# ysnrkdm/subproc

Measured on AMD Instinct MI355X. Metric: env-steps/sec (batched self-play), higher is better.
Workload: dtype u64

## Files before the change

subproc_amd/csrc/bitboard.hpp:

```cpp
#pragma once
#include <hip/hip_runtime.h>
#include <stdint.h>

namespace oth {

typedef uint64_t u64;
typedef uint32_t u32;

constexpr u64 INNER_FILES = 0x7E7E7E7E7E7E7E7Eull;

template <int TT>
__device__ __forceinline__ u64 bitop3(u64 a, u64 b, u64 c) {
    const u32 hi = (u32)__builtin_amdgcn_bitop3_b32((u32)(a >> 32), (u32)(b >> 32), (u32)(c >> 32), TT);
    const u32 lo = (u32)__builtin_amdgcn_bitop3_b32((u32)a, (u32)b, (u32)c, TT);
    return ((u64)hi << 32) | lo;
}
__device__ __forceinline__ u64 bfi(u64 m, u64 a, u64 b) { return bitop3<0xCA>(m, a, b); }
__device__ __forceinline__ u64 andn(u64 a, u64 b) { return bitop3<0x30>(a, b, b); }
__device__ __forceinline__ u64 or3(u64 a, u64 b, u64 c) { return bitop3<0xFE>(a, b, c); }
__device__ __forceinline__ u64 and2(u64 a, u64 b) { return bitop3<0xC0>(a, b, b); }
__device__ __forceinline__ u64 or2(u64 a, u64 b) { return bitop3<0xFC>(a, b, b); }
template <int K, bool L>
__device__ __forceinline__ u32 sh32(u32 x) {
    u32 r;
    if (L) asm("v_lshlrev_b32_e64 %0, %2, %1" : "=v"(r) : "v"(x), "i"(K));
    else asm("v_lshrrev_b32_e64 %0, %2, %1" : "=v"(r) : "v"(x), "i"(K));
    return r;
}
template <int S, bool L>
__device__ __forceinline__ u64 sh(u64 x) {
    static_assert(S > 0 && S < 64, "shift amount");
    u64 r;
    if (L) asm("v_lshlrev_b64 %0, %2, %1" : "=v"(r) : "v"(x), "i"(S));
    else asm("v_lshrrev_b64 %0, %2, %1" : "=v"(r) : "v"(x), "i"(S));
    return r;
}

struct PairProp {
    u64 pro, p2L, p4L, p2R, p4R;
};
template <int S>
__device__ __forceinline__ PairProp pair_prop(u64 pro) {
    PairProp q;
    q.pro = pro;
    q.p2L = and2(pro, sh<S, true>(pro));
    q.p4L = and2(q.p2L, sh<2 * S, true>(q.p2L));
    q.p2R = sh<S, false>(q.p2L);
    q.p4R = sh<3 * S, false>(q.p4L);
    return q;
}

template <int K, bool L>
__device__ __forceinline__ u64 ks_step(u64 gen, u64 pro) {
    if constexpr (K >= 32) {
        u32 lo = (u32)gen, hi = (u32)(gen >> 32);
        if (L) {
            const u32 s = K == 32 ? lo : sh32<(K == 32 ? 1 : K - 32), true>(lo);
            hi = (u32)__builtin_amdgcn_bitop3_b32((u32)(pro >> 32), s, hi, 0xCA);
        } else {
            const u32 s = K == 32 ? hi : sh32<(K == 32 ? 1 : K - 32), false>(hi);
            lo = (u32)__builtin_amdgcn_bitop3_b32((u32)pro, s, lo, 0xCA);
        }
        return ((u64)hi << 32) | lo;
    } else {
        return bfi(pro, sh<K, L>(gen), gen);
    }
}

template <int S, bool L>
__device__ __forceinline__ u64 ks(u64 gen, const PairProp& q) {
    gen = ks_step<S, L>(gen, q.pro);
    gen = ks_step<2 * S, L>(gen, L ? q.p2L : q.p2R);
    gen = ks_step<4 * S, L>(gen, L ? q.p4L : q.p4R);
    return gen;
}

__device__ __forceinline__ u64 lshl1_add(u64 x, u64 y) {
    u64 r;
    asm("v_lshl_add_u64 %0, %1, 1, %2" : "=v"(r) : "v"(x), "v"(y));
    return r;
}
__device__ __forceinline__ u64 add64(u64 x, u64 y) {
    u64 r;
    asm("v_lshl_add_u64 %0, %1, 0, %2" : "=v"(r) : "v"(x), "v"(y));
    return r;
}
__device__ __forceinline__ u64 dec64(u64 x) {
    u64 r;
    asm("v_lshl_add_u64 %0, %1, 0, -1" : "=v"(r) : "v"(x));
    return r;
}
__device__ __forceinline__ u64 east_run(u64 src, u64 Oi) { return andn(Oi, lshl1_add(src, Oi)); }

__device__ __forceinline__ u32 bfrev32(u32 x) {
    u32 r;
    asm("v_bfrev_b32_e64 %0, %1" : "=v"(r) : "v"(x));
    return r;
}
__device__ __forceinline__ u64 rev64(u64 x) { return ((u64)bfrev32((u32)x) << 32) | bfrev32((u32)(x >> 32)); }

struct Position {
    u64 Oi, rOi;
    u64 A[8];
    u64 reach;
    u64 legal;
};

constexpr int kFillOrder = 798;
template <int ORDER = kFillOrder>
__device__ __forceinline__ void analyse(u64 P, u64 O, Position& s) {
    const u64 Oi = and2(O, INNER_FILES);
    s.Oi = Oi;
    s.rOi = rev64(Oi);
    const PairProp v = pair_prop<8>(O), d9 = pair_prop<9>(Oi), d7 = pair_prop<7>(Oi);
    s.A[0] = east_run(P, Oi);
    s.A[1] = rev64(east_run(rev64(P), s.rOi));
    {
        constexpr int order[3] = {ORDER / 100, ORDER / 10 % 10, ORDER % 10};
#pragma unroll
        for (int k = 0; k < 3; k++) {
            if (order[k] == 8) {
                s.A[2] = and2(ks<8, true>(P, v), O);
                s.A[3] = and2(ks<8, false>(P, v), O);
            } else if (order[k] == 9) {
                s.A[4] = and2(ks<9, true>(P, d9), O);
                s.A[5] = and2(ks<9, false>(P, d9), O);
            } else {
                s.A[6] = and2(ks<7, true>(P, d7), O);
                s.A[7] = and2(ks<7, false>(P, d7), O);
            }
        }
    }
    u64 m = or3(sh<1, true>(s.A[0]), sh<1, false>(s.A[1]), sh<8, true>(s.A[2]));
    m = or3(m, sh<8, false>(s.A[3]), sh<9, true>(s.A[4]));
    m = or3(m, sh<9, false>(s.A[5]), sh<7, true>(s.A[6]));
    m = or2(m, sh<7, false>(s.A[7]));
    s.reach = m;
    s.legal = bitop3<0x04>(P, m, O);
}

constexpr int kRayRows = 6;
constexpr int kTabRows = kRayRows + 2;
__host__ __device__ inline u64 ray_from(int sq, int dx, int dy) {
    u64 r = 0;
    int x = sq & 7, y = sq >> 3;
    for (;;) {
        x += dx;
        y += dy;
        if (x < 0 || x > 7 || y < 0 || y > 7) break;
        r |= 1ull << (x + 8 * y);
    }
    return r;
}
__device__ __forceinline__ void ray_table_init(u64* tab) {
    for (int e = threadIdx.x; e < kTabRows * 64; e += blockDim.x) {
        const int row = e >> 6, sq = e & 63;
        const int dx[6] = {0, 1, -1, 0, -1, 1}, dy[6] = {1, 1, 1, -1, -1, -1};
        if (row >= kRayRows) {
            tab[e] = 1ull << (row == kRayRows ? sq : 63 - sq);
            continue;
        }
        const u64 r = ray_from(sq, dx[row], dy[row]);
        tab[e] = row < 3 ? r : rev64(r);
    }
}
__device__ __forceinline__ u64 square_bit(u32 sq, const u64* tab) { return tab[kRayRows * 64 + sq]; }
__device__ __forceinline__ u64 and3(u64 a, u64 b, u64 c) { return bitop3<0x80>(a, b, c); }
__device__ __forceinline__ u64 run_prefix(u64 R, u64 A) {
    const u64 x = andn(R, A);
    return and3(R, A, dec64(x));
}

struct RunSets {
    u64 A1, A3, A5, A7, rA0, rA2, rA4, rA6;
};
__device__ __forceinline__ RunSets run_sets(const Position& s) {
    return RunSets{s.A[1], s.A[3], s.A[5], s.A[7], rev64(s.A[0]), rev64(s.A[2]), rev64(s.A[4]), rev64(s.A[6])};
}

struct Flips {
    u64 f, fr;
};
__device__ __forceinline__ Flips flips_col(u64 mv, const RunSets& r, const u64* col) {
    const u64 rmv = col[(kRayRows + 1) * 64];
    u64 f = bitop3<0xBA>(r.A1, lshl1_add(mv, r.A1), mv);
    u64 fr = bitop3<0xBA>(r.rA0, lshl1_add(rmv, r.rA0), rmv);
    f = or3(f, run_prefix(col[0 * 64], r.A3), run_prefix(col[1 * 64], r.A5));
    f = or2(f, run_prefix(col[2 * 64], r.A7));
    fr = or3(fr, run_prefix(col[3 * 64], r.rA2), run_prefix(col[4 * 64], r.rA4));
    fr = or2(fr, run_prefix(col[5 * 64], r.rA6));
    return Flips{f, rev64(fr)};
}
__device__ __forceinline__ Flips flips_rays(u32 sq, const RunSets& r, const u64* tab) {
    return flips_col(tab[kRayRows * 64 + sq], r, tab + sq);
}
__device__ __forceinline__ void place(u64& X, u64& Y, const Flips& fl) {
    X = or3(X, fl.f, fl.fr);
    Y = bitop3<0x10>(Y, fl.f, fl.fr);
}
__device__ __forceinline__ const u64* ray_col(const u64* tab, u32 off) {
    return reinterpret_cast<const u64*>(reinterpret_cast<const char*>(tab) + off);
}

__device__ __forceinline__ u64 sel_nz(u64 t, u64 x) {
    u32 lo, hi;
    u64 m;
    asm("v_cmp_ne_u64_e64 %2, 0, %3\n\t"
        "s_nop 1\n\t"
        "v_cndmask_b32_e64 %0, 0, %4, %2\n\t"
        "v_cndmask_b32_e64 %1, 0, %5, %2"
        : "=&v"(lo), "=&v"(hi), "=&s"(m)
        : "v"(t), "v"((u32)x), "v"((u32)(x >> 32)));
    return ((u64)hi << 32) | lo;
}
__device__ __forceinline__ u64 ray_flips(u64 mv, u64 R, u64 P, u64 O) {
    const u64 sum = add64(bfi(R, O, ~0ull), mv);
    const u64 run = bitop3<0x20>(R, sum, O);
    return sel_nz(and3(sum, R, P), run);
}

__device__ __forceinline__ void rays_of(u32 sq, u64 (&R)[kRayRows]) {
    const u32 rsq = sq ^ 63u;
    R[0] = 0x0101010101010100ull << sq;
    R[1] = 0x8040201008040200ull << sq;
    R[2] = 0x0002040810204080ull << sq;
    R[3] = 0x0101010101010100ull << rsq;
    R[4] = 0x8040201008040200ull << rsq;
    R[5] = 0x0002040810204080ull << rsq;
}

__device__ __forceinline__ u64 flips_carry(u32 sq, u64 P, u64 O) {
    u64 R[kRayRows];
    rays_of(sq, R);
    const u64 mv = 1ull << sq, rmv = 1ull << (63u - sq);
    const u64 rP = rev64(P), rO = rev64(O);
    const u64 Oi = and2(O, INNER_FILES), rOi = and2(rO, INNER_FILES);
    const u64 se = lshl1_add(mv, Oi), sw = lshl1_add(rmv, rOi);
    u64 f = sel_nz(and2(se, P), andn(Oi, se));
    u64 fr = sel_nz(and2(sw, rP), andn(rOi, sw));
    f = or3(f, ray_flips(mv, R[0], P, O), ray_flips(mv, R[1], P, Oi));
    f = or2(f, ray_flips(mv, R[2], P, Oi));
    fr = or3(fr, ray_flips(rmv, R[3], rP, rO), ray_flips(rmv, R[4], rP, rOi));
    fr = or2(fr, ray_flips(rmv, R[5], rP, rOi));
    return or2(f, rev64(fr));
}

template <int ORDER = kFillOrder>
__device__ __forceinline__ u64 moves(u64 P, u64 O) {
    Position s;
    analyse<ORDER>(P, O, s);
    return s.legal;
}

__device__ __forceinline__ u64 moves_empty_side(u64 black, u64 white) {
    const u64 E = ~(black | white);
    Position s;
    analyse(E, black, s);
    return s.reach & E;
}

__device__ __forceinline__ void kth_table_init(uint8_t* tab) {
    for (int b = threadIdx.x; b < 256; b += blockDim.x) {
        int k = 0;
        for (int i = 0; i < 8; i++)
            if (b >> i & 1) tab[b * 8 + k++] = (uint8_t)i;
        for (; k < 8; k++) tab[b * 8 + k] = 0;
    }
}
__device__ __forceinline__ u32 add_lshl3(u32 a, u32 b) {
    u32 r;
    asm("v_add_lshl_u32 %0, %1, %2, 3" : "=v"(r) : "v"(a), "v"(b));
    return r;
}
template <int S, bool W>
__device__ __forceinline__ void kth_level(u32& k, u32 c, u32& off, u32& w, u32 w_hi) {
    u32 d, k2, o, w2;
    u64 b;
    if (W)
        asm("v_sub_co_u32_e64 %0, %4, %5, %6\n\t"
            "s_nop 1\n\t"
            "v_cndmask_b32_e64 %1, %0, %5, %4\n\t"
            "v_cndmask_b32_e64 %2, %7, 0, %4\n\t"
            "v_cndmask_b32_e64 %3, %9, %8, %4"
            : "=&v"(d), "=&v"(k2), "=&v"(o), "=v"(w2), "=&s"(b)
            : "v"(k), "v"(c), "i"(S), "v"(w), "v"(w_hi));
    else
        asm("v_sub_co_u32_e64 %0, %3, %4, %5\n\t"
            "s_nop 1\n\t"
            "v_cndmask_b32_e64 %1, %0, %4, %3\n\t"
            "v_cndmask_b32_e64 %2, %6, 0, %3"
            : "=&v"(d), "=&v"(k2), "=v"(o), "=&s"(b)
            : "v"(k), "v"(c), "i"(S));
    k = k2;
    off = o;
    if (W) w = w2;
}
__device__ __forceinline__ u32 kth_bit_off(u64 x, u32 k, u32 c_lo, const uint8_t* tab) {
    u32 w = (u32)x, b32, s16, s8;
    kth_level<32, true>(k, c_lo, b32, w, (u32)(x >> 32));
    kth_level<16, false>(k, __popc(w & 0xFFFFu), s16, w, 0u);
    w >>= s16;
    kth_level<8, false>(k, __popc(w & 0xFFu), s8, w, 0u);
    const u32 byte = __builtin_amdgcn_ubfe(w, s8, 8);
    const u32 lvl = (u32)__builtin_amdgcn_bitop3_b32(b32, s16, s8, 0xFE);
    return add_lshl3(lvl, tab[byte * 8u + k]);
}
__device__ __forceinline__ u32 kth_bit_tab(u64 x, u32 k, u32 c_lo, const uint8_t* tab) {
    return kth_bit_off(x, k, c_lo, tab) >> 3;
}

__device__ __forceinline__ u32 kth_bit(u64 x, u32 k) {
    u32 lo = (u32)x, hi = (u32)(x >> 32);
    u32 c = __popc(lo);
    bool up = k >= c;
    u32 w = up ? hi : lo;
    k = up ? k - c : k;
    u32 pos = up ? 32u : 0u;
#pragma unroll
    for (int half = 16; half >= 1; half >>= 1) {
        const u32 mask = (1u << half) - 1u;
        c = __popc(w & mask);
        up = k >= c;
        w = up ? (w >> half) : w;
        k = up ? k - c : k;
        pos += up ? (u32)half : 0u;
    }
    return pos;
}

}
```

subproc_amd/csrc/othello.hip:

```cpp
#include <hip/hip_runtime.h>
#include <stdint.h>
#include <stdlib.h>

#include <algorithm>
#include <climits>
#include <cmath>
#include <atomic>
#include <mutex>

#include "../../include/othello.h"
#include "bitboard.hpp"
#include "td_skey.hpp"

#define OTH_VERSION "subproc_amd 0.1.0 gfx950"

namespace {

using namespace oth;

constexpr u64 OPEN_BLACK = 0x0000000810000000ull;
constexpr u64 OPEN_WHITE = 0x0000001008000000ull;
constexpr int kBlock = 256;

constexpr u64 GOLDEN64 = 0x9E3779B97F4A7C15ull;
__host__ __device__ __forceinline__ u64 mix64(u64 z) {
    z = (z ^ (z >> 30)) * 0xBF58476D1CE4E5B9ull;
    z = (z ^ (z >> 27)) * 0x94D049BB133111EBull;
    return z ^ (z >> 31);
}
__device__ __forceinline__ u64 game_key(u64 S, u64 g) { return mix64(S + g * GOLDEN64); }
constexpr u32 LCG_MUL = 0x915F77F5u;
struct GameRng {
    u32 state, inc;
    __device__ __forceinline__ void init(u64 key) {
        state = (u32)key;
        inc = (u32)(key >> 32) | 1u;
    }
    __device__ __forceinline__ u32 pick(u32 n) {
        state = state * LCG_MUL + inc;
        return __umulhi(state, n);
    }
};
__device__ __forceinline__ u32 pick_legal(u64 legal, GameRng& rng, const uint8_t* kth_tab) {
    const u32 c_lo = __popc((u32)legal);
    return kth_bit_tab(legal, rng.pick(c_lo + __popc((u32)(legal >> 32))), c_lo, kth_tab);
}


__constant__ u64 kRegionMasks[8] = {0x8100000000000081ull, 0x4281000000008142ull, 0x0042000000004200ull,
                                    0x2400810000810024ull, 0x1800008181000018ull, 0x003C424242423C00ull,
                                    0x0000240000240000ull, 0x0000183C3C180000ull};

constexpr int kEvalRow = 12;
constexpr int kEvalTable = OTH_EVAL_PHASES * kEvalRow;
struct EvalWeights {
    int8_t w[OTH_EVAL_WEIGHTS];
};
__device__ __forceinline__ u32 eval_shard(u32 discs) { return discs ? (min(discs, 64u) - 1u) >> 4 : 0u; }
__device__ __forceinline__ void eval_weights_to_lds(const EvalWeights& ew, int* w_s) {
    for (int e = threadIdx.x; e < OTH_EVAL_PHASES * kEvalRow; e += blockDim.x) {
        const int r = e / kEvalRow, c = e % kEvalRow;
        w_s[e] = c < OTH_EVAL_FEATURES ? (int)ew.w[r * OTH_EVAL_FEATURES + c] : 0;
    }
}
__device__ __forceinline__ int eval_mul(int w, int c) { return __mul24(w, c); }
__device__ __forceinline__ int eval_linear(const int* w, u64 mine, u64 mob) {
    int v = eval_mul(w[0], (int)__popcll(mob));
#pragma unroll
    for (int k = 0; k < 8; k++) v += eval_mul(w[1 + k], (int)__popcll(and2(mine, kRegionMasks[k])));
    return v;
}

template <int POLICY>
__device__ __forceinline__ const int* child_row(u64 P, u64 O, const int* w_tab) {
    if (POLICY != OTH_POLICY_EVAL) return w_tab;
    return w_tab + kEvalRow * eval_shard((u32)__popcll(P | O) + 1u);
}
template <int POLICY>
__device__ __forceinline__ u32 child_key(u64 P, u64 O, const RunSets& s, u32 sq, const u64* rays, const int* row) {
    place(P, O, flips_rays(sq, s, rays));
    if (POLICY == OTH_POLICY_GREEDY) return ((u32)__popcll(moves(O, P)) << 6) | sq;
    int w[OTH_EVAL_FEATURES];
#pragma unroll
    for (int j = 0; j < OTH_EVAL_FEATURES; j++) w[j] = row[j];
    const int v = eval_linear(w, P, moves<798>(P, O));
    return ((u32)((1 << 20) - v) << 6) | sq;
}

template <int POLICY>
__device__ __forceinline__ u32 lane_choose(const Position& pos, u64 P, u64 O, const u64* rays, const int* w_tab) {
    u32 best = 0xFFFFFFFFu;
    u64 legal = pos.legal;
    const RunSets s = run_sets(pos);
    const int* row = child_row<POLICY>(P, O, w_tab);
    while (legal) {
        const u32 sq = (u32)__builtin_ctzll(legal);
        legal &= legal - 1;
        best = min(best, child_key<POLICY>(P, O, s, sq, rays, row));
    }
    return best & 63u;
}

struct CoopWave {
    u64 rec[64][10];
    u64 legal[64];
    u32 best[64];
};
__device__ __forceinline__ void wave_sync() {
    __builtin_amdgcn_fence(__ATOMIC_SEQ_CST, "wavefront");
    __builtin_amdgcn_wave_barrier();
}
static_assert(sizeof(RunSets) == 8 * sizeof(u64), "parent record: P, O, RunSets");
__device__ __forceinline__ void load_parent(const u64* r, u64& P, u64& O, RunSets& s) {
    P = r[0];
    O = r[1];
    s = *reinterpret_cast<const RunSets*>(r + 2);
}
__device__ __forceinline__ u32 wave_incl_scan(u32 x) {
    x += (u32)__builtin_amdgcn_update_dpp(0, (int)x, 0x111, 0xf, 0xf, false);
    x += (u32)__builtin_amdgcn_update_dpp(0, (int)x, 0x112, 0xf, 0xf, false);
    x += (u32)__builtin_amdgcn_update_dpp(0, (int)x, 0x114, 0xf, 0xf, false);
    x += (u32)__builtin_amdgcn_update_dpp(0, (int)x, 0x118, 0xf, 0xf, false);
    x += (u32)__builtin_amdgcn_update_dpp(0, (int)x, 0x142, 0xa, 0xf, false);
    x += (u32)__builtin_amdgcn_update_dpp(0, (int)x, 0x143, 0xc, 0xf, false);
    return x;
}
template <int POLICY>
__device__ u32 coop_choose(bool need, u64 P, u64 O, u32 tbl, const Position& pos, CoopWave& cw, const u64* rays,
                           const int* w_s, const uint8_t* kth_tab, u32 lane, u32 cap) {
    auto publish = [&] {
        u64* r = cw.rec[lane];
        r[0] = P;
        r[1] = O;
        RunSets rs = run_sets(pos);
        if (POLICY == OTH_POLICY_EVAL) rs.A1 |= (u64)(tbl & 1u);
        *reinterpret_cast<RunSets*>(r + 2) = rs;
    };
    constexpr bool kFirst = POLICY == OTH_POLICY_GREEDY;
    if (kFirst && need) publish();
    if (cap == 0) return need ? lane_choose<POLICY>(pos, P, O, rays, w_s + (tbl ? kEvalTable : 0)) : 64u;
    const u64 legal = need ? pos.legal : 0ull;
    const u32 cnt = (u32)__popcll(legal);
    const u32 incl = wave_incl_scan(cnt);
    const u32 T = (u32)__builtin_amdgcn_readlane((int)incl, 63);
    const u32 R = (T + 63u) >> 6;
    cw.legal[lane] = legal;
    if (need) {
        if (!kFirst) publish();
        cw.best[lane] = 0xFFFFFFFFu;
    }
    const u32 t0 = R * lane, cnt_mine = t0 < T ? min(R, T - t0) : 0u;
    const u32 excl = incl - cnt;
    const u64 with_moves = __ballot(cnt != 0);
    u32 p = 0;
#pragma unroll
    for (u32 step = 32; step >= 1; step >>= 1)
        if ((u32)__shfl((int)excl, (int)(p + step)) <= t0) p += step;
    const u32 k0 = t0 - (u32)__shfl((int)excl, (int)p);
    wave_sync();
    u64 m = 0, Pp = 0, Op = 0;
    RunSets ps = {};
    const int* row = w_s;
    auto enter = [&](u32 q) {
        load_parent(cw.rec[q], Pp, Op, ps);
        row = child_row<POLICY>(Pp, Op, w_s + ((ps.A1 & 1ull) ? kEvalTable : 0));
    };
    if (cnt_mine) {
        m = cw.legal[p];
        enter(p);
        if (k0) m &= ~0ull << kth_bit_tab(m, k0, (u32)__popc((u32)m), kth_tab);
    }
    for (u32 r = 0; r < cnt_mine; r++) {
        if (m == 0) {
            p = (u32)__ffsll((unsigned long long)(with_moves & (~0ull << (p + 1)))) - 1u;
            m = cw.legal[p];
            enter(p);
        }
        const u32 sq = (u32)__builtin_ctzll(m);
        m &= m - 1;
        atomicMin(&cw.best[p], child_key<POLICY>(Pp, Op, ps, sq, rays, row));
    }
    wave_sync();
    return need ? cw.best[lane] & 63u : 64u;
}

__device__ __forceinline__ int lane_id() { return __lane_id(); }
__device__ __forceinline__ u64 moves_of(u64 P, u64 O) { return moves(P, O); }

__global__ __launch_bounds__(kBlock) void reset_kernel(u64* __restrict__ boards, uint8_t* __restrict__ turn,
                                                       uint8_t* __restrict__ nturn, int64_t n) {
    const int64_t i = (int64_t)blockIdx.x * kBlock + threadIdx.x;
    if (i >= n) return;
    reinterpret_cast<ulonglong2*>(boards)[i] = make_ulonglong2(OPEN_BLACK, OPEN_WHITE);
    if (turn) turn[i] = OTH_BLACK;
    if (nturn) nturn[i] = 0;
}

__device__ __forceinline__ u64 legal_any(u64 bl, u64 wh, u32 t) {
    if (t == OTH_BLACK) return moves(bl, wh);
    if (t == OTH_WHITE) return moves(wh, bl);
    if (t == 0) return moves_empty_side(bl, wh);
    return 0ull;
}

struct StepOut {
    u64 bl, wh, flips;
    u32 t;
    int ret;
};
__device__ __forceinline__ StepOut put_s_any(u64 bl, u64 wh, u32 t, u32 c) {
    const u64 occ = bl | wh;
    const bool black = t == OTH_BLACK, white = t == OTH_WHITE;
    const u64 own = black ? bl : (white ? wh : (t == 0 ? ~occ : 0ull));
    const u64 opp = black ? wh : bl;
    StepOut o{bl, wh, 0ull, t, -1};
    if (c == OTH_PASS) {
        o.ret = 0;
    } else if (c < 64 && !(occ >> c & 1ull)) {
        const u64 f = flips_carry(c, own, opp);
        if (f) {
            const u64 mv = 1ull << c;
            o.ret = __popcll(f);
            o.flips = f;
            if (black) {
                o.bl = or3(bl, f, mv);
                o.wh = andn(wh, f);
            } else if (white) {
                o.wh = or3(wh, f, mv);
                o.bl = andn(bl, f);
            } else {
                o.bl = andn(bl, f);
            }
        }
    }
    if (o.ret >= 0) o.t = black ? OTH_WHITE : OTH_BLACK;
    return o;
}

__global__ __launch_bounds__(kBlock) void legal_kernel(const u64* __restrict__ boards,
                                                       const uint8_t* __restrict__ turn, u64* __restrict__ legal,
                                                       int64_t n) {
    const int64_t i = (int64_t)blockIdx.x * kBlock + threadIdx.x;
    if (i >= n) return;
    const ulonglong2 b = reinterpret_cast<const ulonglong2*>(boards)[i];
    legal[i] = legal_any(b.x, b.y, turn[i]);
}

__device__ __forceinline__ void step_board(int64_t i, ulonglong2 b, u32 t, u32 mvc, u64* boards_out, uint8_t* turn_out,
                                           u64* __restrict__ flips_out,
                                           u64* __restrict__ legal_next, int8_t* __restrict__ ret_out,
                                           uint8_t* __restrict__ nturn) {
    u64 nb, nw, f = 0, lg = 0;
    u32 t_out;
    int r = -1;
    if (t == OTH_BLACK || t == OTH_WHITE) {
        const bool black = t == OTH_BLACK;
        u64 P = black ? b.x : b.y;
        u64 O = black ? b.y : b.x;
        if (mvc == OTH_PASS) {
            r = 0;
        } else if (mvc < 64) {
            const u64 mv = 1ull << mvc;
            if (!((P | O) & mv)) {
                f = flips_carry(mvc, P, O);
                if (f) {
                    r = __popcll(f);
                    P = or3(P, f, mv);
                    O = andn(O, f);
                }
            }
        }
        const bool moved = r >= 0;
        t_out = moved ? (t ^ 3u) : t;
        if (legal_next) {
            const u64 nP = moved ? O : P, nO = moved ? P : O;
            lg = moves(nP, nO);
        }
        nb = black ? P : O;
        nw = black ? O : P;
    } else {
        const StepOut o = put_s_any(b.x, b.y, t, mvc);
        nb = o.bl;
        nw = o.wh;
        f = o.flips;
        r = o.ret;
        t_out = o.t;
        if (legal_next) lg = legal_any(nb, nw, t_out);
    }
    if (legal_next) __builtin_nontemporal_store(lg, legal_next + i);
    if (boards_out) {
        __builtin_nontemporal_store(nb, boards_out + 2 * i);
        __builtin_nontemporal_store(nw, boards_out + 2 * i + 1);
    }
    if (turn_out) __builtin_nontemporal_store((uint8_t)t_out, turn_out + i);
    if (flips_out) __builtin_nontemporal_store(f, flips_out + i);
    if (ret_out) __builtin_nontemporal_store((int8_t)r, ret_out + i);
    if (nturn && r >= 0) nturn[i] = (uint8_t)(nturn[i] + 1);
}

constexpr int kStepPerThread = 1;
__global__ __launch_bounds__(kBlock) void step_kernel(const u64* boards_in, const uint8_t* turn_in,
                                                      const uint8_t* __restrict__ move, u64* boards_out,
                                                      uint8_t* turn_out, u64* __restrict__ flips_out,
                                                      u64* __restrict__ legal_next, int8_t* __restrict__ ret_out,
                                                      uint8_t* __restrict__ nturn, int64_t n) {
    const int64_t i0 = (int64_t)blockIdx.x * kBlock + threadIdx.x, stride = (int64_t)gridDim.x * kBlock;
    ulonglong2 b[kStepPerThread];
    u32 t[kStepPerThread], mvc[kStepPerThread];
#pragma unroll
    for (int j = 0; j < kStepPerThread; j++) {
        const int64_t i = i0 + j * stride;
        if (i < n) {
            b[j] = reinterpret_cast<const ulonglong2*>(boards_in)[i];
            t[j] = turn_in[i];
            mvc[j] = move[i];
            asm volatile("" ::"v"(t[j]), "v"(mvc[j]));
        }
    }
#pragma unroll
    for (int j = 0; j < kStepPerThread; j++) {
        const int64_t i = i0 + j * stride;
        if (i < n) step_board(i, b[j], t[j], mvc[j], boards_out, turn_out, flips_out, legal_next, ret_out, nturn);
    }
}

__device__ __forceinline__ bool step_on_board(int64_t x, int64_t d, int k, int64_t& out) {
    int64_t t;
    return !__builtin_mul_overflow(d, (int64_t)k, &t) && !__builtin_add_overflow(x, t, &out) && out >= 0 && out < 8;
}
__global__ __launch_bounds__(kBlock) void hands_kernel(const u64* __restrict__ own, const u64* __restrict__ hostile,
                                                       const int64_t* __restrict__ xs, const int64_t* __restrict__ ys,
                                                       const int64_t* __restrict__ dxs,
                                                       const int64_t* __restrict__ dys,
                                                       uint8_t* __restrict__ count, int64_t n) {
    const int64_t i = (int64_t)blockIdx.x * kBlock + threadIdx.x;
    if (i >= n) return;
    const u64 mine = own[i], opp = hostile[i];
    const int64_t x = xs[i], y = ys[i], dx = dxs[i], dy = dys[i];
    int run = 0;
    for (int k = 1; k < 9; k++) {
        int64_t nx, ny;
        const bool on = step_on_board(x, dx, k, nx) && step_on_board(y, dy, k, ny);
        const u64 bit = on ? 1ull << (nx + 8 * ny) : 0ull;
        if (opp & bit) {
            run = k;
        } else {
            if (!(mine & bit)) run = 0;
            break;
        }
    }
    count[i] = (uint8_t)run;
}

__global__ __launch_bounds__(kBlock) void result_kernel(const u64* __restrict__ boards, uint8_t* __restrict__ nb,
                                                        uint8_t* __restrict__ nw, int8_t* __restrict__ diff,
                                                        uint8_t* __restrict__ terminal, int64_t n) {
    const int64_t i = (int64_t)blockIdx.x * kBlock + threadIdx.x;
    if (i >= n) return;
    const ulonglong2 b = reinterpret_cast<const ulonglong2*>(boards)[i];
    const int cb = __popcll(b.x), cw = __popcll(b.y);
    if (nb) nb[i] = (uint8_t)cb;
    if (nw) nw[i] = (uint8_t)cw;
    if (diff) diff[i] = (int8_t)(cb - cw);
    if (terminal) terminal[i] = (moves(b.x, b.y) == 0 && moves(b.y, b.x) == 0) ? 1 : 0;
}


struct RolloutArgs {
    const u64* start;
    const uint8_t* start_turn;
    u64 seed_state;
    u64 game_id0;
    int n_random;
    u64* final_boards;
    int8_t* diff;
    uint8_t* plies;
    uint8_t* moves;
    long long* hist;
    int64_t n;
    unsigned long long* work;
    u64 last_ticket;
    u32 coop_cap;
    EvalWeights ew[2];
    u32 n_rand_a, n_rand_b;
    int swap;
    uint8_t* a_black;
    u32 handoff_k;
};

constexpr u32 kHandoffK = 16;
constexpr u32 kHandoffKMax = 16;
constexpr int kPoolCap = 64 + (int)kHandoffKMax;
struct Parked {
    u64 P, O;
    u32 state, inc;
    u32 g;
    u32 bits;
};
static_assert(sizeof(Parked) == 32, "two 16-B LDS accesses per parked game");
constexpr u64 kParkedGame = ~0ull;

constexpr int kRecStride = OTH_MOVES_STRIDE + 4;
constexpr int kRecWaveBytes = 64 * kRecStride;
constexpr size_t rec_stage_bytes(int policy, bool record) {
    return record && policy == OTH_POLICY_RANDOM ? (size_t)(kBlock / 64) * kRecWaveBytes : 0;
}

constexpr int kRandomFillOrder = 789;
constexpr int rollout_waves_per_simd(int policy) { return policy == OTH_POLICY_GREEDY ? 5 : 4; }
template <int POLICY, bool RECORD, bool RUNNER = false>
__global__ __launch_bounds__(kBlock, rollout_waves_per_simd(POLICY)) void rollout_kernel(RolloutArgs a) {
    __shared__ unsigned long long hist_s[OTH_HIST_BINS];
    __shared__ uint8_t kth_tab[256 * 8];
    __shared__ u64 rays[kTabRows * 64];
    __shared__ int w_s[POLICY == OTH_POLICY_EVAL ? 2 * kEvalTable : 1];
    __shared__ CoopWave coop[POLICY == OTH_POLICY_RANDOM ? 1 : kBlock / 64];
    constexpr bool kPool = POLICY == OTH_POLICY_RANDOM && !RECORD && !RUNNER;
    __shared__ Parked pool_s[kPool ? kBlock / 64 : 1][kPool ? kPoolCap : 1];
    for (int k = threadIdx.x; k < OTH_HIST_BINS; k += kBlock) hist_s[k] = 0;
    kth_table_init(kth_tab);
    ray_table_init(rays);
    if (POLICY == OTH_POLICY_EVAL) {
        eval_weights_to_lds(a.ew[0], w_s);
        eval_weights_to_lds(a.ew[1], w_s + kEvalTable);
    }
    __syncthreads();

    const int lane = lane_id();
    const u64 n = (u64)a.n;
    u64 plies_sum = 0;
    constexpr bool kRecStage = RECORD && POLICY == OTH_POLICY_RANDOM;
    extern __shared__ u32 rec_dyn[];
    uint8_t* const rec_wave = reinterpret_cast<uint8_t*>(rec_dyn) + (threadIdx.x >> 6) * kRecWaveBytes;
    uint8_t* const rec_row = rec_wave + lane * kRecStride;

    Parked* const pool = pool_s[kPool ? threadIdx.x >> 6 : 0];
    u32 parked = 0;
    bool exhausted = false;
    (void)pool;
    (void)exhausted;
    for (;;) {
        bool from_pool = false;
        u64 base = 0;
        if (kPool && parked >= 64u) {
            from_pool = true;
        } else if (!kPool || !exhausted) {
            if (lane == 0) {
                base = atomicAdd(a.work, 64ull);
                if (base == a.last_ticket) atomicExch(a.work, 0ull);
            }
            base = __shfl(base, 0);
            if (base >= n) {
                if (!kPool || parked == 0u) break;
                exhausted = true;
                from_pool = true;
            }
        } else {
            if (parked == 0u) break;
            from_pool = true;
        }

        u64 g = base + lane;
        bool active = !from_pool && g < n;
        u64 P = OPEN_BLACK, O = OPEN_WHITE;
        u32 side = OTH_BLACK, ply = 0;
        bool passed = false;
        GameRng rng;
        if (active) {
            rng.init(game_key(a.seed_state, a.game_id0 + g));
            if (a.start) {
                const ulonglong2 s0 = reinterpret_cast<const ulonglong2*>(a.start)[g];
                side = a.start_turn ? a.start_turn[g] : OTH_BLACK;
                side = side == OTH_WHITE ? OTH_WHITE : OTH_BLACK;
                P = side == OTH_BLACK ? s0.x : s0.y;
                O = side == OTH_BLACK ? s0.y : s0.x;
            }
            if (RECORD && !kRecStage) {
                uint4* mrec = reinterpret_cast<uint4*>(a.moves + g * OTH_MOVES_STRIDE);
#pragma unroll
                for (int q = 0; q < OTH_MOVES_STRIDE / 16; q++) mrec[q] = make_uint4(~0u, ~0u, ~0u, ~0u);
            }
        }
        if constexpr (kRecStage) {
#pragma unroll
            for (int q = 0; q < OTH_MOVES_STRIDE / 4; q++) reinterpret_cast<u32*>(rec_row)[q] = ~0u;
        }
        auto rec_put = [&](u32 i, uint8_t code) {
            if (i >= OTH_MOVES_STRIDE) return;
            if constexpr (kRecStage) rec_row[i] = code;
            else a.moves[g * OTH_MOVES_STRIDE + i] = code;
        };

        if constexpr (POLICY == OTH_POLICY_RANDOM) {
            bool b0 = side == OTH_BLACK;
            u32 discs0 = RECORD ? 0u : (u32)__popcll(P | O);
            u32 npass = 0;
            if (kPool && from_pool) {
                const u32 take = min(parked, 64u);
                active = (u32)lane < take;
                if (active) {
                    const Parked e = pool[parked - take + lane];
                    P = e.P;
                    O = e.O;
                    rng.state = e.state;
                    rng.inc = e.inc;
                    g = e.g;
                    b0 = e.bits & 1u;
                    passed = (e.bits >> 1) & 1u;
                    discs0 = (e.bits >> 2) & 0x7fu;
                    npass = e.bits >> 9;
                }
                parked -= take;
            }
            const u32 hand_k = __builtin_amdgcn_readfirstlane(kPool && !from_pool ? a.handoff_k : 0u);
            const u32 parked0 = __builtin_amdgcn_readfirstlane(parked);
            (void)hand_k;
            (void)parked0;
            auto ply_of = [&](u64& X, u64& Y) -> bool {
                Position pos;
                analyse<kRandomFillOrder>(X, Y, pos);
                const u64 legal = pos.legal;
                const u32 c_lo = __popc((u32)legal), nl = c_lo + __popc((u32)(legal >> 32));
                if (nl == 0) {
                    if (passed || (X | Y) == ~0ull) {
                        if (passed) npass--;
                        return true;
                    }
                    if (RECORD) rec_put(npass, OTH_PASS);
                    passed = true;
                    npass++;
                    return false;
                }
                passed = false;
                const u32 off = kth_bit_off(legal, rng.pick(nl), c_lo, kth_tab);
                const u64* col = ray_col(rays, off);
                const Flips f = flips_col(col[kRayRows * 64], run_sets(pos), col);
                if (RECORD) {
                    rec_put(npass, (uint8_t)(off >> 3));
                    npass++;
                }
                place(X, Y, f);
                return false;
            };
            if (active) {
                for (;;) {
                    if (ply_of(P, O)) break;
                    if (ply_of(O, P)) break;
                    if (kPool) {
                        const u64 live = __ballot(1);
                        if ((u32)__popcll(live) <= hand_k) {
                            const u32 rank = __builtin_amdgcn_mbcnt_hi((u32)(live >> 32),
                                                                       __builtin_amdgcn_mbcnt_lo((u32)live, 0u));
                            pool[parked0 + rank] = Parked{P, O, rng.state, rng.inc, (u32)g,
                                                          (u32)b0 | (u32)passed << 1 | discs0 << 2 | npass << 9};
                            g = kParkedGame;
                            break;
                        }
                    }
                }
            }
            if (kPool) {
                const u64 pm = __ballot(active && g == kParkedGame);
                parked = parked0 + (u32)__popcll(pm);
                if (g == kParkedGame) active = false;
            }
            if (active) {
                const u32 ply = RECORD ? npass : (u32)__popcll(P | O) - discs0 + npass;
                if (RECORD) rec_put(ply, 0xFF);
                const u64 bl = b0 ? P : O, wh = b0 ? O : P;
                const int d = __popcll(bl) - __popcll(wh);
                if (a.final_boards) reinterpret_cast<ulonglong2*>(a.final_boards)[g] = make_ulonglong2(bl, wh);
                if (a.diff) a.diff[g] = (int8_t)d;
                if (a.plies) a.plies[g] = (uint8_t)ply;
                atomicAdd(&hist_s[d + 64], 1ull);
                atomicAdd(&hist_s[d > 0 ? 129 : (d < 0 ? 130 : 131)], 1ull);
                plies_sum += ply;
            }
        } else {
            u32 rem_b = 0, rem_w = 0, tbl_black = 0;
            if (RUNNER && active) {
                const bool ab = !(a.swap && rng.pick(2) == 1u);
                rem_b = ab ? a.n_rand_a : a.n_rand_b;
                rem_w = ab ? a.n_rand_b : a.n_rand_a;
                tbl_black = ab ? 0u : 1u;
                if (a.a_black) a.a_black[g] = (uint8_t)ab;
            }
            while (__ballot(active)) {
                bool moving = false, choose = false;
                u32 sq = 0;
                Position pos;
                if (active) {
                    analyse(P, O, pos);
                    const u64 legal = pos.legal;
                    if (legal == 0) {
                        if (passed || (P | O) == ~0ull) {
                            const u64 bl = side == OTH_BLACK ? P : O, wh = side == OTH_BLACK ? O : P;
                            const int d = __popcll(bl) - __popcll(wh);
                            u64 gt = g;
                            if (POLICY == OTH_POLICY_GREEDY) asm volatile("" : "+v"(gt));
                            if (a.final_boards)
                                reinterpret_cast<ulonglong2*>(a.final_boards)[gt] = make_ulonglong2(bl, wh);
                            if (a.diff) a.diff[gt] = (int8_t)d;
                            if (a.plies) a.plies[gt] = (uint8_t)ply;
                            atomicAdd(&hist_s[d + 64], 1ull);
                            atomicAdd(&hist_s[d > 0 ? 129 : (d < 0 ? 130 : 131)], 1ull);
                            if (POLICY == OTH_POLICY_GREEDY) atomicAdd(&hist_s[132], (unsigned long long)ply);
                            else plies_sum += ply;
                            active = false;
                        } else {
                            passed = true;
                            const u64 t = P;
                            P = O;
                            O = t;
                            side ^= 3u;
                        }
                    } else {
                        if (passed) {
                            if (RECORD) rec_put(ply, OTH_PASS);
                            ply++;
                            passed = false;
                            if (RUNNER) {
                                const u32 rx = side == OTH_BLACK ? rem_w : rem_b;
                                if (rx) (void)rng.pick(rx);
                            }
                        }
                        moving = true;
                        if (RUNNER) {
                            const u32 r = side == OTH_BLACK ? rem_b : rem_w;
                            if (r && rng.pick(r) == 0u) {
                                sq = pick_legal(legal, rng, kth_tab);
                                if (side == OTH_BLACK) rem_b--;
                                else rem_w--;
                            } else {
                                choose = true;
                            }
                        } else if ((int)ply >= a.n_random) {
                            choose = true;
                        } else {
                            sq = pick_legal(legal, rng, kth_tab);
                        }
                    }
                }
                CoopWave& cw = coop[__builtin_amdgcn_readfirstlane(threadIdx.x >> 6)];
                auto play = [&](u32 m, const RunSets& rs) {
                    if (RECORD) rec_put(ply, (uint8_t)m);
                    place(P, O, flips_rays(m, rs, rays));
                    const u64 np = O;
                    O = P;
                    P = np;
                    side ^= 3u;
                    ply++;
                };
                constexpr bool kFromRecord = POLICY == OTH_POLICY_GREEDY;
                if (kFromRecord && moving && !choose) play(sq, run_sets(pos));
                if (__ballot(choose)) {
                    const u32 tbl = side == OTH_BLACK ? tbl_black : tbl_black ^ 1u;
                    const u32 c = coop_choose<POLICY>(choose, P, O, tbl, pos, cw, rays, w_s, kth_tab, (u32)lane,
                                                      a.coop_cap);
                    if (choose) {
                        sq = c;
                        if (kFromRecord) {
                            u64 Pr, Or;
                            RunSets rs;
                            load_parent(cw.rec[lane], Pr, Or, rs);
                            play(c, rs);
                        }
                    }
                }
                if (!kFromRecord && moving) play(sq, run_sets(pos));
            }
        }
        if constexpr (kRecStage) {
            wave_sync();
            const int nvalid = (int)min<u64>(64, n - base);
            for (int c = lane; c < nvalid * (OTH_MOVES_STRIDE / 16); c += 64) {
                const int j = c / (OTH_MOVES_STRIDE / 16), part = c % (OTH_MOVES_STRIDE / 16);
                const u32* src = reinterpret_cast<const u32*>(rec_wave + j * kRecStride + part * 16);
                reinterpret_cast<uint4*>(a.moves + (base + j) * OTH_MOVES_STRIDE)[part] =
                    make_uint4(src[0], src[1], src[2], src[3]);
            }
            wave_sync();
        }
    }

    for (int off = 32; off >= 1; off >>= 1) plies_sum += __shfl_xor(plies_sum, off);
    if (lane == 0) atomicAdd(&hist_s[132], (unsigned long long)plies_sum);
    __syncthreads();
    if (a.hist)
        for (int k = threadIdx.x; k < OTH_HIST_BINS; k += kBlock)
            if (hist_s[k]) atomicAdd((unsigned long long*)&a.hist[k], hist_s[k]);
}

__global__ __launch_bounds__(kBlock) void sample_midgame_kernel(u64 S, u64 index0, u64* __restrict__ boards,
                                                                uint8_t* __restrict__ turn,
                                                                uint8_t* __restrict__ nturn,
                                                                uint8_t* __restrict__ move, int64_t n) {
    const int64_t j = (int64_t)blockIdx.x * kBlock + threadIdx.x;
    if (j >= n) return;
    const u64 i = index0 + (u64)j;
    for (u64 attempt = 0;; attempt++) {
        GameRng rng;
        rng.init(game_key(S, i ^ (attempt << 48)));
        const u32 target = 10 + rng.pick(40);
        u64 P = OPEN_BLACK, O = OPEN_WHITE;
        u32 side = OTH_BLACK, ply = 0;
        for (;;) {
            const u64 legal = moves(P, O);
            if (legal == 0 && moves(O, P) == 0) break;
            if (ply >= target && legal) {
                const u32 sq = kth_bit(legal, rng.pick((u32)__popcll(legal)));
                reinterpret_cast<ulonglong2*>(boards)[j] =
                    side == OTH_BLACK ? make_ulonglong2(P, O) : make_ulonglong2(O, P);
                turn[j] = (uint8_t)side;
                if (nturn) nturn[j] = (uint8_t)ply;
                move[j] = (uint8_t)sq;
                return;
            }
            if (legal) {
                const u32 sq = kth_bit(legal, rng.pick((u32)__popcll(legal)));
                const u64 mv = 1ull << sq;
                const u64 f = flips_carry(sq, P, O);
                P = or3(P, f, mv);
                O = andn(O, f);
            }
            const u64 t = P;
            P = O;
            O = t;
            side ^= 3u;
            ply++;
        }
    }
}

constexpr int kReplayBurst = 8;
constexpr int kReplayStage = kBlock * OTH_POS_STRIDE;
constexpr u32 kTurnEscape = 0x7f;
static_assert(kReplayStage % 16 == 0, "block stage = whole 16-B chunks");

__device__ __forceinline__ void load_move_record(const uint8_t* row, bool vec, u64 (&R)[OTH_MOVES_STRIDE / 8]) {
    if (vec) {
        const ulonglong2* r2 = reinterpret_cast<const ulonglong2*>(row);
#pragma unroll
        for (int j = 0; j < OTH_MOVES_STRIDE / 16; j++) {
            const ulonglong2 v = r2[j];
            R[2 * j] = v.x;
            R[2 * j + 1] = v.y;
        }
    } else {
#pragma unroll
        for (int j = 0; j < OTH_MOVES_STRIDE / 8; j++) {
            u64 w = 0;
#pragma unroll 1
            for (int k = 0; k < 8; k++) w |= (u64)row[8 * j + k] << (8 * k);
            R[j] = w;
        }
    }
}

constexpr int kReplayBursts = (OTH_POS_STRIDE + 7 + kReplayBurst - 1) / kReplayBurst;
constexpr int kXHalf = kReplayBurst / 2;
constexpr int kReplayPackedRows = 72;
constexpr int kReplayStagePacked = kBlock * kReplayPackedRows + 16;

template <bool PACKED>
__global__ __launch_bounds__(kBlock, PACKED ? 4 : 3) void replay_kernel(const u64* __restrict__ start,
                                                        const uint8_t* __restrict__ start_turn,
                                                        const uint8_t* __restrict__ moves,
                                                        const uint8_t* __restrict__ plies,
                                                        const int64_t* __restrict__ row_off, u64* __restrict__ pos,
                                                        uint8_t* __restrict__ pos_turn, uint8_t* __restrict__ pos_end,
                                                        int64_t n, int vec_moves, int vec_out) {
    extern __shared__ uint4 replay_stage4[];
    __shared__ uint4 xrow[kBlock * kXHalf];
    __shared__ unsigned long long xaddr[kBlock];
    __shared__ u32 xmask[kBlock];
    uint8_t* stage = reinterpret_cast<uint8_t*>(replay_stage4);
    const bool staged = pos_turn || pos_end;
    const int64_t blk0 = (int64_t)blockIdx.x * kBlock;
    const int nb = (int)min<int64_t>(kBlock, n - blk0);
    const int lane = threadIdx.x;
    const int wl = lane & 63, wbase = lane & ~63;
    int64_t base = blk0 * OTH_POS_STRIDE, bytes = (int64_t)nb * OTH_POS_STRIDE;
    if (PACKED && staged) {
        __shared__ long long rows_lo[kBlock / 64], rows_hi[kBlock / 64];
        long long lo = LLONG_MAX, hi = LLONG_MIN;
        if (threadIdx.x < nb) {
            lo = row_off[blk0 + threadIdx.x];
            hi = lo + min<int>(plies[blk0 + threadIdx.x], OTH_MOVES_STRIDE) + 1;
        }
        for (int off = 32; off >= 1; off >>= 1) {
            lo = min(lo, __shfl_xor(lo, off));
            hi = max(hi, __shfl_xor(hi, off));
        }
        if ((threadIdx.x & 63) == 0) {
            rows_lo[threadIdx.x >> 6] = lo;
            rows_hi[threadIdx.x >> 6] = hi;
        }
        __syncthreads();
        for (int w = 0; w < kBlock / 64; w++) {
            lo = min(lo, rows_lo[w]);
            hi = max(hi, rows_hi[w]);
        }
        base = lo;
        bytes = hi - lo;
    } else if (PACKED) {
        base = row_off[blk0];
    }
    const int64_t base_al = PACKED ? (base & ~(int64_t)15) : base;
    const int lead = (int)(base - base_al);
    const int64_t span = lead + bytes;
    const bool direct = PACKED && staged && span > kReplayStagePacked;
    if (staged && !direct) {
        for (int c = lane; c < (PACKED ? kReplayStagePacked : kReplayStage) / 16; c += kBlock)
            replay_stage4[c] = make_uint4(0, 0, 0, 0);
        __syncthreads();
    }
    const bool live = lane < nb;
    const int64_t i = blk0 + (live ? lane : 0);
    u64 bl = OPEN_BLACK, wh = OPEN_WHITE;
    u32 t = OTH_BLACK;
    if (live && start) {
        const ulonglong2 s0 = reinterpret_cast<const ulonglong2*>(start)[i];
        bl = s0.x;
        wh = s0.y;
        t = start_turn ? start_turn[i] : OTH_BLACK;
    }
    const int np = live ? min<int>(plies[i], OTH_MOVES_STRIDE) : -1;
    u64 R[OTH_MOVES_STRIDE / 8];
    if (live) load_move_record(moves + i * OTH_MOVES_STRIDE, vec_moves != 0, R);
    else
#pragma unroll
        for (int j = 0; j < OTH_MOVES_STRIDE / 8; j++) R[j] = 0;
    const int64_t row0 = PACKED ? (live ? row_off[i] : base) : i * OTH_POS_STRIDE;
    ulonglong2* out = reinterpret_cast<ulonglong2*>(pos) + row0;
    uint8_t* st = stage + (direct ? 0 : row0 - base_al);
    auto put_te = [&](int p, u32 v, u32 t_full) {
        if (!direct) {
            st[p] = (uint8_t)v;
        } else {
            if (pos_turn) pos_turn[row0 + p] = (uint8_t)t_full;
            if (pos_end) pos_end[row0 + p] = (uint8_t)(v >> 7);
        }
    };
    const int s = (int)(row0 & 7);
    int bursts = kReplayBursts;
    if (PACKED) {
        bursts = live ? (np + 1 + s + kReplayBurst - 1) / kReplayBurst : 0;
        for (int off = 32; off >= 1; off >>= 1) bursts = max(bursts, __shfl_xor(bursts, off));
    }
    u64 prev = 0, cur = R[0];
    for (int bi = 0; bi < bursts; bi++) {
        const int p0 = 8 * bi - s;
        const u64 win = s ? (cur << (8 * s)) | (prev >> (64 - 8 * s)) : cur;
#pragma unroll
        for (int h = 0; h < kReplayBurst / kXHalf; h++) {
          u32 valid = 0;
#pragma unroll
          for (int kk = 0; kk < kXHalf; kk++) {
            const int k = h * kXHalf + kk;
            const int p = p0 + k;
            ulonglong2 row = make_ulonglong2(0ull, 0ull);
            if (p >= 0 && p <= np) {
                row = make_ulonglong2(bl, wh);
                const u32 c = (u32)(win >> (8 * k)) & 0xffu;
                const bool fast = t == OTH_BLACK || t == OTH_WHITE;
                if (pos_end && fast) {
                    const bool black = t == OTH_BLACK;
                    u64 P = black ? bl : wh, O = black ? wh : bl;
                    u64 f = 0;
                    if (p < np && c < 64 && !((P | O) >> c & 1ull)) f = flips_carry(c, P, O);
                    u32 e = 0;
                    if (!f && moves_of(P, O) == 0) e = moves_of(O, P) == 0;
                    put_te(p, t | (e << 7), t);
                    if (f) {
                        P = or3(P, f, 1ull << c);
                        O = andn(O, f);
                        bl = black ? P : O;
                        wh = black ? O : P;
                        t ^= 3u;
                    } else if (p < np && c == OTH_PASS) {
                        t ^= 3u;
                    }
                } else {
                if (staged) {
                    u32 e = 0;
                    if (pos_end && moves_of(bl, wh) == 0) e = moves_of(wh, bl) == 0;
                    put_te(p, min(t, kTurnEscape) | (e << 7), t);
                }
                if (p < np && !fast) {
                    const StepOut o = put_s_any(bl, wh, t, c);
                    bl = o.bl;
                    wh = o.wh;
                    t = o.t;
                } else if (p < np) {
                    if (c == OTH_PASS) {
                        t ^= 3u;
                    } else if (c < 64) {
                        const bool black = t == OTH_BLACK;
                        u64 P = black ? bl : wh, O = black ? wh : bl;
                        const u64 mm = 1ull << c;
                        if (!((P | O) & mm)) {
                            const u64 f = flips_carry(c, P, O);
                            if (f) {
                                P |= f | mm;
                                O = andn(O, f);
                                bl = black ? P : O;
                                wh = black ? O : P;
                                t ^= 3u;
                            }
                        }
                    }
                }
                }
            }
            xrow[lane * kXHalf + kk] = make_uint4((u32)row.x, (u32)(row.x >> 32), (u32)row.y, (u32)(row.y >> 32));
            valid |= (live && p >= 0 && p < (PACKED ? np + 1 : OTH_POS_STRIDE) ? 1u : 0u) << kk;
          }
            xaddr[lane] = reinterpret_cast<unsigned long long>(out + (p0 + h * kXHalf));
            xmask[lane] = valid;
            wave_sync();
#pragma unroll
            for (int j = 0; j < 64 / (64 / kXHalf); j++) {
                const int src = wbase + j * (64 / kXHalf) + wl / kXHalf, c = wl % kXHalf;
                if (xmask[src] >> c & 1u)
                    reinterpret_cast<uint4*>(xaddr[src])[c] = xrow[src * kXHalf + c];
            }
            wave_sync();
        }
        prev = cur;
#pragma unroll
        for (int j = 0; j < OTH_MOVES_STRIDE / 8 - 1; j++) R[j] = R[j + 1];
        R[OTH_MOVES_STRIDE / 8 - 1] = 0;
        cur = R[0];
    }
    if (!staged || direct) return;
    __syncthreads();
    auto game_of = [&](int64_t q) -> int64_t {
        if (!PACKED) return blk0 + q / OTH_POS_STRIDE;
        const int64_t row = base_al + q;
        for (int k = 0; k < nb; k++) {
            const int64_t r0 = row_off[blk0 + k];
            if (row >= r0 && row <= r0 + min<int>(plies[blk0 + k], OTH_MOVES_STRIDE)) return blk0 + k;
        }
        return blk0;
    };
    if (vec_out) {
        for (int c = lane; c * 16 < span; c += kBlock) {
            const uint4 v = replay_stage4[c];
            u32 w[4] = {v.x, v.y, v.z, v.w};
            u32 tw[4], ew[4];
            bool esc = false;
#pragma unroll
            for (int q = 0; q < 4; q++) {
                tw[q] = w[q] & 0x7f7f7f7fu;
                ew[q] = (w[q] >> 7) & 0x01010101u;
                esc |= ((tw[q] + 0x01010101u) & 0x80808080u) != 0;
            }
            const int64_t q0 = (int64_t)c * 16;
            if (esc) {
#pragma unroll 1
                for (int q = 0; q < 16; q++) {
                    if (q0 + q < lead || q0 + q >= span) continue;
                    const u32 byte = w[q >> 2] >> (8 * (q & 3)) & 0xffu;
                    if ((byte & kTurnEscape) != kTurnEscape) continue;
                    const u32 tb = start_turn[game_of(q0 + q)];
                    tw[q >> 2] = (tw[q >> 2] & ~(0xffu << (8 * (q & 3)))) | (tb << (8 * (q & 3)));
                }
            }
            const int64_t g0 = base_al + q0;
            if (q0 >= lead && q0 + 16 <= span) {
                if (pos_turn) *reinterpret_cast<uint4*>(pos_turn + g0) = make_uint4(tw[0], tw[1], tw[2], tw[3]);
                if (pos_end) *reinterpret_cast<uint4*>(pos_end + g0) = make_uint4(ew[0], ew[1], ew[2], ew[3]);
// ... 1150 lines not shown
```

Before: 217.1 billion.

## Fold Kogge-Stone fill reach into analyse and derive flip runs from generators

Reworks the directional fill so each Kogge-Stone pass returns its generator and first shifted source. The reach mask is accumulated incrementally with one bitop3 per direction, and the separate and-with-O run sets are dropped. Flip computation now masks the generator against P (or reversed P) inside run_prefix, so analyse does less work per position. The default fill order changes, PairProp construction moves inside each direction, and sched barriers are inserted between directions to limit register pressure. The cost is extra fields (rP) in the structs and slightly more work in the flip and parent-record paths.

```diff
diff --git a/subproc_amd/csrc/bitboard.hpp b/subproc_amd/csrc/bitboard.hpp
--- a/subproc_amd/csrc/bitboard.hpp
+++ b/subproc_amd/csrc/bitboard.hpp
@@ -67,12 +67,19 @@
     }
 }
 
+struct Fill {
+    u64 G, PS;
+};
 template <int S, bool L>
-__device__ __forceinline__ u64 ks(u64 gen, const PairProp& q) {
-    gen = ks_step<S, L>(gen, q.pro);
+__device__ __forceinline__ Fill ks(u64 src, const PairProp& q) {
+    static_assert(S < 32, "the first step's shifted source is a whole 64-bit shift");
+    Fill f;
+    f.PS = sh<S, L>(src);
+    u64 gen = bfi(q.pro, f.PS, src);
     gen = ks_step<2 * S, L>(gen, L ? q.p2L : q.p2R);
     gen = ks_step<4 * S, L>(gen, L ? q.p4L : q.p4R);
-    return gen;
+    f.G = gen;
+    return f;
 }
 
 __device__ __forceinline__ u64 lshl1_add(u64 x, u64 y) {
@@ -101,40 +108,50 @@
 
 struct Position {
     u64 Oi, rOi;
-    u64 A[8];
+    u64 rP;
+    u64 A[2];
+    u64 G[8];
     u64 reach;
     u64 legal;
 };
 
-constexpr int kFillOrder = 798;
+template <int S, bool L>
+__device__ __forceinline__ u64 fill_reach(u64 P, const PairProp& q, u64& m) {
+    const Fill f = ks<S, L>(P, q);
+    m = bitop3<0xF4>(m, sh<S, L>(f.G), f.PS);
+    return f.G;
+}
+
+constexpr int kFillOrder = 789;
 template <int ORDER = kFillOrder>
 __device__ __forceinline__ void analyse(u64 P, u64 O, Position& s) {
     const u64 Oi = and2(O, INNER_FILES);
     s.Oi = Oi;
     s.rOi = rev64(Oi);
-    const PairProp v = pair_prop<8>(O), d9 = pair_prop<9>(Oi), d7 = pair_prop<7>(Oi);
+    s.rP = rev64(P);
     s.A[0] = east_run(P, Oi);
-    s.A[1] = rev64(east_run(rev64(P), s.rOi));
+    s.A[1] = rev64(east_run(s.rP, s.rOi));
+    u64 m = or2(sh<1, true>(s.A[0]), sh<1, false>(s.A[1]));
     {
         constexpr int order[3] = {ORDER / 100, ORDER / 10 % 10, ORDER % 10};
 #pragma unroll
         for (int k = 0; k < 3; k++) {
             if (order[k] == 8) {
-                s.A[2] = and2(ks<8, true>(P, v), O);
-                s.A[3] = and2(ks<8, false>(P, v), O);
+                const PairProp v = pair_prop<8>(O);
+                s.G[2] = fill_reach<8, true>(P, v, m);
+                s.G[3] = fill_reach<8, false>(P, v, m);
             } else if (order[k] == 9) {
-                s.A[4] = and2(ks<9, true>(P, d9), O);
-                s.A[5] = and2(ks<9, false>(P, d9), O);
+                const PairProp d9 = pair_prop<9>(Oi);
+                s.G[4] = fill_reach<9, true>(P, d9, m);
+                s.G[5] = fill_reach<9, false>(P, d9, m);
             } else {
-                s.A[6] = and2(ks<7, true>(P, d7), O);
-                s.A[7] = and2(ks<7, false>(P, d7), O);
+                const PairProp d7 = pair_prop<7>(Oi);
+                s.G[6] = fill_reach<7, true>(P, d7, m);
+                s.G[7] = fill_reach<7, false>(P, d7, m);
             }
+            __builtin_amdgcn_sched_barrier(0);
         }
     }
-    u64 m = or3(sh<1, true>(s.A[0]), sh<1, false>(s.A[1]), sh<8, true>(s.A[2]));
-    m = or3(m, sh<8, false>(s.A[3]), sh<9, true>(s.A[4]));
-    m = or3(m, sh<9, false>(s.A[5]), sh<7, true>(s.A[6]));
-    m = or2(m, sh<7, false>(s.A[7]));
     s.reach = m;
     s.legal = bitop3<0x04>(P, m, O);
 }
@@ -166,29 +183,40 @@
 }
 __device__ __forceinline__ u64 square_bit(u32 sq, const u64* tab) { return tab[kRayRows * 64 + sq]; }
 __device__ __forceinline__ u64 and3(u64 a, u64 b, u64 c) { return bitop3<0x80>(a, b, c); }
-__device__ __forceinline__ u64 run_prefix(u64 R, u64 A) {
-    const u64 x = andn(R, A);
-    return and3(R, A, dec64(x));
-}
-
+__device__ __forceinline__ u64 run_prefix(u64 R, u64 G, u64 P) {
+    const u64 x = bitop3<0xB0>(R, G, P);
+    return and3(R, G, dec64(x));
+}
+
+struct Runs {
+    u64 A1, G3, G5, G7, rA0, rG2, rG4, rG6;
+};
 struct RunSets {
-    u64 A1, A3, A5, A7, rA0, rA2, rA4, rA6;
-};
-__device__ __forceinline__ RunSets run_sets(const Position& s) {
-    return RunSets{s.A[1], s.A[3], s.A[5], s.A[7], rev64(s.A[0]), rev64(s.A[2]), rev64(s.A[4]), rev64(s.A[6])};
+    Runs r;
+    u64 P, rP;
+};
+__device__ __forceinline__ RunSets run_sets(u64 P, const Position& s) {
+    return RunSets{{s.A[1], s.G[3], s.G[5], s.G[7], rev64(s.A[0]), rev64(s.G[2]), rev64(s.G[4]), rev64(s.G[6])},
+                   P, s.rP};
+}
+__device__ __forceinline__ RunSets run_sets_parent(u64 P, const Position& s) {
+    return RunSets{{s.A[1], s.G[3], s.G[5], s.G[7], rev64(s.A[0]), rev64(andn(s.G[2], P)), rev64(andn(s.G[4], P)),
+                    rev64(andn(s.G[6], P))},
+                   P, 0ull};
 }
 
 struct Flips {
     u64 f, fr;
 };
-__device__ __forceinline__ Flips flips_col(u64 mv, const RunSets& r, const u64* col) {
+__device__ __forceinline__ Flips flips_col(u64 mv, const RunSets& s, const u64* col) {
+    const Runs& r = s.r;
     const u64 rmv = col[(kRayRows + 1) * 64];
     u64 f = bitop3<0xBA>(r.A1, lshl1_add(mv, r.A1), mv);
     u64 fr = bitop3<0xBA>(r.rA0, lshl1_add(rmv, r.rA0), rmv);
-    f = or3(f, run_prefix(col[0 * 64], r.A3), run_prefix(col[1 * 64], r.A5));
-    f = or2(f, run_prefix(col[2 * 64], r.A7));
-    fr = or3(fr, run_prefix(col[3 * 64], r.rA2), run_prefix(col[4 * 64], r.rA4));
-    fr = or2(fr, run_prefix(col[5 * 64], r.rA6));
+    f = or3(f, run_prefix(col[0 * 64], r.G3, s.P), run_prefix(col[1 * 64], r.G5, s.P));
+    f = or2(f, run_prefix(col[2 * 64], r.G7, s.P));
+    fr = or3(fr, run_prefix(col[3 * 64], r.rG2, s.rP), run_prefix(col[4 * 64], r.rG4, s.rP));
+    fr = or2(fr, run_prefix(col[5 * 64], r.rG6, s.rP));
     return Flips{f, rev64(fr)};
 }
 __device__ __forceinline__ Flips flips_rays(u32 sq, const RunSets& r, const u64* tab) {
diff --git a/subproc_amd/csrc/othello.hip b/subproc_amd/csrc/othello.hip
--- a/subproc_amd/csrc/othello.hip
+++ b/subproc_amd/csrc/othello.hip
@@ -83,7 +83,7 @@
     int w[OTH_EVAL_FEATURES];
 #pragma unroll
     for (int j = 0; j < OTH_EVAL_FEATURES; j++) w[j] = row[j];
-    const int v = eval_linear(w, P, moves<798>(P, O));
+    const int v = eval_linear(w, P, moves<789>(P, O));
     return ((u32)((1 << 20) - v) << 6) | sq;
 }
 
@@ -91,7 +91,7 @@
 __device__ __forceinline__ u32 lane_choose(const Position& pos, u64 P, u64 O, const u64* rays, const int* w_tab) {
     u32 best = 0xFFFFFFFFu;
     u64 legal = pos.legal;
-    const RunSets s = run_sets(pos);
+    const RunSets s = run_sets_parent(P, pos);
     const int* row = child_row<POLICY>(P, O, w_tab);
     while (legal) {
         const u32 sq = (u32)__builtin_ctzll(legal);
@@ -110,11 +110,13 @@
     __builtin_amdgcn_fence(__ATOMIC_SEQ_CST, "wavefront");
     __builtin_amdgcn_wave_barrier();
 }
-static_assert(sizeof(RunSets) == 8 * sizeof(u64), "parent record: P, O, RunSets");
+static_assert(sizeof(Runs) == 8 * sizeof(u64), "parent record: P, O, Runs");
 __device__ __forceinline__ void load_parent(const u64* r, u64& P, u64& O, RunSets& s) {
     P = r[0];
     O = r[1];
-    s = *reinterpret_cast<const RunSets*>(r + 2);
+    s.r = *reinterpret_cast<const Runs*>(r + 2);
+    s.P = P;
+    s.rP = 0;
 }
 __device__ __forceinline__ u32 wave_incl_scan(u32 x) {
     x += (u32)__builtin_amdgcn_update_dpp(0, (int)x, 0x111, 0xf, 0xf, false);
@@ -132,9 +134,9 @@
         u64* r = cw.rec[lane];
         r[0] = P;
         r[1] = O;
-        RunSets rs = run_sets(pos);
+        Runs rs = run_sets_parent(P, pos).r;
         if (POLICY == OTH_POLICY_EVAL) rs.A1 |= (u64)(tbl & 1u);
-        *reinterpret_cast<RunSets*>(r + 2) = rs;
+        *reinterpret_cast<Runs*>(r + 2) = rs;
     };
     constexpr bool kFirst = POLICY == OTH_POLICY_GREEDY;
     if (kFirst && need) publish();
@@ -163,7 +165,7 @@
     const int* row = w_s;
     auto enter = [&](u32 q) {
         load_parent(cw.rec[q], Pp, Op, ps);
-        row = child_row<POLICY>(Pp, Op, w_s + ((ps.A1 & 1ull) ? kEvalTable : 0));
+        row = child_row<POLICY>(Pp, Op, w_s + ((ps.r.A1 & 1ull) ? kEvalTable : 0));
     };
     if (cnt_mine) {
         m = cw.legal[p];
@@ -534,7 +536,7 @@
                 passed = false;
                 const u32 off = kth_bit_off(legal, rng.pick(nl), c_lo, kth_tab);
                 const u64* col = ray_col(rays, off);
-                const Flips f = flips_col(col[kRayRows * 64], run_sets(pos), col);
+                const Flips f = flips_col(col[kRayRows * 64], run_sets(X, pos), col);
                 if (RECORD) {
                     rec_put(npass, (uint8_t)(off >> 3));
                     npass++;
@@ -652,7 +654,7 @@
                     ply++;
                 };
                 constexpr bool kFromRecord = POLICY == OTH_POLICY_GREEDY;
-                if (kFromRecord && moving && !choose) play(sq, run_sets(pos));
+                if (kFromRecord && moving && !choose) play(sq, run_sets_parent(P, pos));
                 if (__ballot(choose)) {
                     const u32 tbl = side == OTH_BLACK ? tbl_black : tbl_black ^ 1u;
                     const u32 c = coop_choose<POLICY>(choose, P, O, tbl, pos, cw, rays, w_s, kth_tab, (u32)lane,
@@ -667,7 +669,7 @@
                         }
                     }
                 }
-                if (!kFromRecord && moving) play(sq, run_sets(pos));
+                if (!kFromRecord && moving) play(sq, run_sets_parent(P, pos));
             }
         }
         if constexpr (kRecStage) {
```

New measurement: 224.1 billion, median of 6. 1.03x the previous value.
